# mickgordinier/DPX_GPU_Genomics_Project

Hardware: AMD Instinct MI355X
Metric: GCUPS (higher is better)
Workload: dtype int16; 1 GPU; LSW 10000-pair 1024x1024 batch per GPU, int16 score matrix written to HBM; algorithm=LSW, pairs_per_gpu=10000, query_len=1024, reference_len=1024, match=3, mismatch=-1, gap=-2, parallelism=1 GPU, world_size=1, tune_placement=True, cells_per_gpu=10485760000, matrix_bytes_per_gpu=22261760000, precondition_fills=78, kernel=k_linear_fill_pk, rows_per_lane=16

## Files before the change

### dpx_gpu_genomics_project_amd/csrc/dpx_capi.cpp

```cpp
#include <algorithm>
#include <cstdlib>
#include <cstring>
#include <mutex>
#include <string>
#include <vector>

#include "dpx_batch.h"

static std::mutex g_mu;
static int g_device = -1;

int dpx_host::bind_device(int device) {
    if (device < 0) {
        if (g_device < 0) {
            int rc = dpx_init(0);
            if (rc != DPX_OK) return rc;
        }
        device = g_device;
    }
    HIP_TRY(hipSetDevice(device));
    t_device = device;
    return DPX_OK;
}

// ... 525 lines not shown
    }
    if (r.dirs) return dpx_launch_fill_dir(b->dirArgs, b->kernelAlgo, b->R, s);
    if (r.split) return dpx_launch_fill_split(b->args, b->kernelAlgo, b->R, b->splitWaves, b->splitLds, s);
    hipStream_t side = s;
    bool forked = false;
    if (r.second != DPX_SECOND_NONE && r.main != DPX_MAIN_NONE && b->sideStream && b->evFork && b->evJoin) {
        hipError_t e = hipEventRecord(b->evFork, s);
        if (e == hipSuccess) e = hipStreamWaitEvent(b->sideStream, b->evFork, 0);
        if (e != hipSuccess) return e;
        side = b->sideStream;
        forked = true;
    }
    hipError_t e = launch_main(b, r, side);
    switch (e == hipSuccess ? r.second : DPX_SECOND_NONE) {
    case DPX_SECOND_NONE: break;
    case DPX_SECOND_PACKED: e = dpx_launch_fill_packed(b->pkArgs, b->kernelAlgo, b->R, b->pkLdsBytes, s); break;
    case DPX_SECOND_BANDED_PACKED: e = dpx_launch_banded_packed(b->pkArgs, b->R, b->pkLdsBytes, s); break;
    case DPX_SECOND_LANES:
        if (r.scoreTable) {
            dpx_subst_args ta = {b->pkArgs, table_ref(b)};
            ta.f.ldsPerWave = (uint32_t)dpx_plan_scoretab_lanes_lds(*b);
            e = dpx_launch_scoretab_lanes(ta, b->kernelAlgo, b->R, s);
            break;
        }
        e = dpx_launch_fill_lanes(b->pkArgs, b->kernelAlgo, b->R, b->store, b->pkLdsBytes, s);
        break;
    case DPX_SECOND_LANES_PK: e = dpx_launch_fill_lanes_packed(b->pkArgs, b->kernelAlgo, b->pkLdsBytes, s); break;
    }
    if (forked) {
        hipError_t j = hipEventRecord(b->evJoin, side);
        if (j == hipSuccess) j = hipStreamWaitEvent(s, b->evJoin, 0);
// ... 193 lines not shown
            len += snprintf(buf + len, cap - (size_t)len, "%s%.3f", k ? "," : "", r.candidatesMs[k]);
        if (r.candidatesMs.empty() && (size_t)len < cap) len += snprintf(buf + len, cap - (size_t)len, "untimed");
        if ((size_t)len < cap) len += snprintf(buf + len, cap - (size_t)len, " pool_fill_ms=");
        for (size_t k = 0; k < r.fillMs.size() && (size_t)len < cap; k++)
            len += snprintf(buf + len, cap - (size_t)len, "%s%.3f", k ? "," : "", r.fillMs[k]);
        if (r.fillMs.empty() && (size_t)len < cap) len += snprintf(buf + len, cap - (size_t)len, "unshopped");
        if (!r.kinds.empty() && (size_t)len < cap) {
            len += snprintf(buf + len, cap - (size_t)len, " pool_kinds=");
            for (size_t k = 0; k < r.kinds.size() && (size_t)len < cap; k++) len += snprintf(buf + len, cap - (size_t)len, "%s%s", k ? "," : "", r.kinds[k].c_str());
        }
        if (!r.ranges.empty() && (size_t)len < cap) {
            len += snprintf(buf + len, cap - (size_t)len, " pool_ranges=");
            for (size_t k = 0; k < r.ranges.size() && (size_t)len < cap; k++) len += snprintf(buf + len, cap - (size_t)len, "%s%s", k ? "," : "", r.ranges[k].c_str());
        }
    } else if (!b->dMat && len > 0 && (size_t)len < cap) len += snprintf(buf + len, cap - (size_t)len, " pool_addr=0x0");
    return DPX_OK;
}

int dpx_batch_info(dpx_batch *b, size_t *numPairs, uint64_t *cells, uint64_t *matrixBytes, uint64_t *algorithmicBytes) {
    if (!b) return DPX_ERR_INVALID;
    if (numPairs) *numPairs = b->numPairs;
    if (cells) *cells = b->cells;
    if (matrixBytes) *matrixBytes = b->matElems * sizeof(int16_t);
    if (algorithmicBytes) *algorithmicBytes = b->algBytes;
    return DPX_OK;
}


int dpx_align_batch(const dpx_params *params, const char *sequences, size_t numBytes, const dpx_seq_pair *pairs,
                    size_t numPairs, int32_t *scores, int32_t *endRow, int32_t *endCol, int16_t **H, int16_t **I,
// ... 44 lines not shown
```

### dpx_gpu_genomics_project_amd/csrc/dpx_host.cpp

```cpp
#include "dpx_host.h"

#include <cstdlib>
#include <cstring>
#include <mutex>

namespace dpx_host {

int hip_fail(hipError_t e, const char *what) {
    t_err = std::string(what) + ": " + hipGetErrorString(e);
    (void)hipGetLastError();
    return e == hipErrorOutOfMemory ? DPX_ERR_NOMEM : DPX_ERR_HIP;
}

static std::mutex g_knobsMu;
static Knobs g_knobs;
void refresh_knobs() {
    auto num = [](const char *name, int unset) { const char *e = getenv(name); return e ? atoi(e) : unset; };
    Knobs k;
    k.rowsPerLane = num("DPX_R", 0);
    k.packed = num("DPX_PACKED", -1);
    k.lanes = num("DPX_LANES", -1);
    k.lanesPk = num("DPX_LANES_PK", -1);
    k.split = num("DPX_SPLIT", -1);
    k.rowTags = num("DPX_ROW_TAGS", -1);
    k.rampLines = num("DPX_RAMP_LINES", -1);
    k.wavesPerBlock = num("DPX_WPB", 0);
    k.group = num("DPX_GROUP", 0);
    k.tbWalk = num("DPX_TB_WALK", -1);
    k.poolProbe = num("DPX_POOL_PROBE", -1);
    { const char *e = getenv("DPX_POOL"); k.poolMalloc = e && !strcmp(e, "malloc"); }
    { const long v = num("DPX_POOL_CHUNK_MB", 0); k.poolChunkBytes = v > 0 ? (size_t)v << 20 : 0; }
    { const char *e = getenv("DPX_POOL_GUARD"); k.poolGuard = !e ? 0 : !strcmp(e, "selftest") ? 2 : 1; }
    k.trace = getenv("DPX_TRACE") != nullptr;
    k.traceVmm = getenv("DPX_TRACE_VMM") != nullptr;
    std::lock_guard<std::mutex> lk(g_knobsMu);
    g_knobs = k;
}
Knobs knobs() { std::lock_guard<std::mutex> lk(g_knobsMu); return g_knobs; }

// ... 2 lines not shown
```

### dpx_gpu_genomics_project_amd/csrc/dpx_kernels.h

```cpp
#ifndef DPX_KERNELS_H
#define DPX_KERNELS_H

#include <hip/hip_runtime.h>
#include <stdint.h>

#include "dpx_layout.h"

#define DPX_K_LNW 0
#define DPX_K_LSW 1
#define DPX_K_ANW 2
#define DPX_K_BSW 3
#define DPX_K_ASW 4
#define DPX_K_BASW 5
#define DPX_K_ASG 6
#define DPX_K_BANW 7
#define DPX_K_BAXT 10


typedef struct dpx_fill_args {
    const char *seq;
    const dpx_pair_dev *pairs;
    const int32_t *order;
    const dpx_wave_desc *waves;
    int32_t numPairs;
// ... 6 lines not shown
    uint32_t ldsRefOff;
    uint32_t ldsQryOff;
    uint32_t ldsBufStride;
    int32_t rowTags;
    int32_t rampLines;
} dpx_fill_args;

hipError_t dpx_launch_fill(const dpx_fill_args &a, int algo, int R, bool store, size_t ldsBytes, hipStream_t stream);
hipError_t dpx_launch_fill_lanes(const dpx_fill_args &a, int algo, int R, bool store, size_t ldsBytes, hipStream_t stream);
hipError_t dpx_launch_affine_fill(const dpx_fill_args &a, int algo, int R, bool store, size_t ldsBytes, hipStream_t stream);
hipError_t dpx_launch_affine_lanes(const dpx_fill_args &a, int algo, int R, bool store, size_t ldsBytes, hipStream_t stream);
hipError_t dpx_launch_bsw_fill(const dpx_fill_args &a, int C, bool store, size_t ldsBytes, hipStream_t stream);
hipError_t dpx_launch_fill_lanes_packed(const dpx_fill_args &a, int algo, size_t ldsBytes, hipStream_t stream);
hipError_t dpx_launch_fill_split(const dpx_fill_args &a, int algo, int R, int waves, size_t ldsBytes, hipStream_t stream);
hipError_t dpx_launch_banded_packed(const dpx_fill_args &a, int C, size_t ldsBytes, hipStream_t stream);
hipError_t dpx_launch_fill_packed(const dpx_fill_args &a, int algo, int R, size_t ldsBytes, hipStream_t stream);
hipError_t dpx_launch_export(const int16_t *mat, const dpx_pair_dev &pr, int algo, int R, int planes, int plane, int gapOpen,
                             int gapExtend, int band, int16_t *out, hipStream_t stream);
hipError_t dpx_launch_traceback(const dpx_fill_args &a, int numPairs, int algo, int R, int planes, int walk,
                                const uint64_t *tbOff, char *tb, int32_t *tbLen, hipStream_t stream);
size_t dpx_out_scan_tiles(size_t numPairs);
hipError_t dpx_launch_output(const dpx_pair_dev *pairs, const int32_t *score, const int32_t *tbLen, const uint64_t *tbOff, const char *tb,
                             int numPairs, unsigned long long firstNumber, unsigned long long *tileSums, unsigned long long *outOff, char *out,
                             bool scanOnly, bool compactOnly, hipStream_t stream);
hipError_t dpx_launch_basw_fill(const dpx_fill_args &a, int C, bool store, size_t ldsBytes, hipStream_t stream);
hipError_t dpx_launch_basw_export(const int16_t *mat, const dpx_pair_dev &pr, int plane, int band, int16_t *out, hipStream_t stream);
hipError_t dpx_launch_basw_traceback(const dpx_fill_args &a, int numPairs, int walk, const uint64_t *tbOff, char *tb, int32_t *tbLen,
                                     hipStream_t stream);
hipError_t dpx_launch_banw_fill(const dpx_fill_args &a, int C, bool store, size_t ldsBytes, hipStream_t stream);
hipError_t dpx_launch_banw_export(const int16_t *mat, const dpx_pair_dev &pr, int plane, int band, int gapOpen, int gapExtend, int16_t *out,
                                  hipStream_t stream);
// ... 44 lines not shown
```

### dpx_gpu_genomics_project_amd/csrc/dpx_kernels.hip

```cpp
#include <hip/hip_runtime.h>
#include <stdint.h>

#include <type_traits>

#include "dpx_fill_common.hpp"
#include "dpx_kernels.h"
#include "dpx_layout.h"
#include "dpx_prims.hpp"

namespace {

using dpx::pack_lo16;
using dpx::wave_shr1;
using dpx::wave_shl1;
using dpx::s16x2;
using dpx::u16x2;
using dpx::as_s16x2;
using dpx::as_u16x2;
using dpx::as_u32;
using namespace dpx_dev;
using namespace dpx_fill;

template <int R, bool LOCAL>
struct LinState {
// ... 615 lines not shown
        __builtin_amdgcn_fence(__ATOMIC_RELEASE, "workgroup");
        int arrived = 0;
        if (lane == 0) arrived = __hip_atomic_fetch_add(&ctrl[16], 1, __ATOMIC_ACQ_REL, __HIP_MEMORY_SCOPE_WORKGROUP);
        arrived = __builtin_amdgcn_readfirstlane(arrived);
        if (arrived == W - 1 && lane == 0) {
            int bv = 0, br = 0, bc = 0;
            for (int k = 0; k < W; k++) {
                const int v = __hip_atomic_load(&result[4 * k], __ATOMIC_RELAXED, __HIP_MEMORY_SCOPE_WORKGROUP);
                if (v > bv) { bv = v; br = result[4 * k + 1]; bc = result[4 * k + 2]; }
            }
            a.score[p] = bv; a.endRow[p] = bv > 0 ? br : 0; a.endCol[p] = bv > 0 ? bc : 0;
        }
    }
}

template <int R>
struct PkState {
    uint32_t Hl[R];
    uint32_t qc[R];
    uint32_t rmax[R];
    uint32_t rcol[R];
    uint32_t dtop;
    uint32_t keyA, keyB;
};

template <int R, int TAG>
__device__ __forceinline__ uint32_t pk_row_tag(uint32_t h) {
    static_assert(TAG >= 0 && TAG < R && R <= 16, "inline constants");
    uint32_t r;
    asm("v_pk_mad_u16 %0, %1, %2, %3 op_sel_hi:[1,0,0]" : "=v"(r) : "v"(h), "n"(R), "n"(TAG));
    return r;
}
template <int R>
__device__ __forceinline__ uint32_t pk_row_tag_of(uint32_t h, const int r) {
#define DPX_TAG_CASE(k) case k: if constexpr (k < R) return pk_row_tag<R, (k < R ? R - 1 - k : 0)>(h); else return 0u;
    switch (r) {
        DPX_TAG_CASE(0) DPX_TAG_CASE(1) DPX_TAG_CASE(2) DPX_TAG_CASE(3) DPX_TAG_CASE(4) DPX_TAG_CASE(5) DPX_TAG_CASE(6) DPX_TAG_CASE(7)
        DPX_TAG_CASE(8) DPX_TAG_CASE(9) DPX_TAG_CASE(10) DPX_TAG_CASE(11) DPX_TAG_CASE(12) DPX_TAG_CASE(13) DPX_TAG_CASE(14) DPX_TAG_CASE(15)
    default: return 0u;
    }
#undef DPX_TAG_CASE
}

template <int R>
__device__ __forceinline__ void store_tile_pk(int16_t *dstA, int16_t *dstB, const uint32_t (&v)[R]) {
    if constexpr (R == 2) {
        *reinterpret_cast<uint32_t *>(dstA) = pk_hi16(v[0], v[1]);
        *reinterpret_cast<uint32_t *>(dstB) = pack_lo16((int)v[0], (int)v[1]);
    } else if constexpr (R == 4) {
        uint2 a, b;
        a.x = pk_hi16(v[0], v[1]); a.y = pk_hi16(v[2], v[3]);
        b.x = pack_lo16((int)v[0], (int)v[1]); b.y = pack_lo16((int)v[2], (int)v[3]);
        *reinterpret_cast<uint2 *>(dstA) = a;
        *reinterpret_cast<uint2 *>(dstB) = b;
    } else {
#pragma unroll
        for (int q = 0; q < R / 8; q++) {
            uint4 a, b;
            a.x = pk_hi16(v[8 * q + 0], v[8 * q + 1]); a.y = pk_hi16(v[8 * q + 2], v[8 * q + 3]);
            a.z = pk_hi16(v[8 * q + 4], v[8 * q + 5]); a.w = pk_hi16(v[8 * q + 6], v[8 * q + 7]);
            b.x = pack_lo16((int)v[8 * q + 0], (int)v[8 * q + 1]); b.y = pack_lo16((int)v[8 * q + 2], (int)v[8 * q + 3]);
            b.z = pack_lo16((int)v[8 * q + 4], (int)v[8 * q + 5]); b.w = pack_lo16((int)v[8 * q + 6], (int)v[8 * q + 7]);
            *reinterpret_cast<uint4 *>(dstA + q * 512) = a;
            *reinterpret_cast<uint4 *>(dstB + q * 512) = b;
        }
    }
}

template <int R, bool LOCAL, bool MASKED, bool WHOLE, bool TAGS = false, bool PARTIAL = false>
__device__ __forceinline__ void pk_step(PkState<R> &st, const int t, const int lane, const int n, const bool laneHasRows, const int nrows,
                                        const uint32_t matchP, const uint32_t negDeltaP, const uint32_t gapP, const uint32_t e0,
                                        const uint32_t rcP, uint32_t *edge, const bool writeEdge, int16_t *tileA, int16_t *tileB,
                                        const int storeLanes, const int rampLines) {
    const int j = t - lane + 1;
    const uint32_t upin = (uint32_t)wave_shr1((int)st.Hl[R - 1], (int)e0);
    bool active = true;
    if constexpr (MASKED) active = laneHasRows && (j >= 1) && (j <= n);
    if (active) {
        uint32_t u = upin, d = st.dtop;
        const uint32_t onesP = 0x00010001u;
        const uint32_t negj = 0xFFFFu - (uint32_t)j;
        uint32_t colMax = 0u;
#pragma unroll
        for (int r = 0; r < R; r++) {
            const uint32_t left = st.Hl[r];
            const uint32_t differs = dpx::pk_min_u16_raw(st.qc[r] ^ rcP, onesP);
            const s16x2 sc = as_s16x2(dpx::pk_mad_i16_raw(differs, negDeltaP, matchP));
            s16x2 h;
            if constexpr (LOCAL && TAGS) {
                h = dpx::pk_max(pk_gap_sat(u, left, gapP), (s16x2)(as_s16x2(d) + sc));
            } else {
                const s16x2 g = dpx::pk_max(as_s16x2(u), as_s16x2(left)) + as_s16x2(gapP);
                h = dpx::pk_max(g, (s16x2)(as_s16x2(d) + sc));
                if constexpr (LOCAL) h = dpx::pk_max(h, as_s16x2(0u));
            }
            d = left;
            u = as_u32(h);
            st.Hl[r] = u;
            if constexpr (LOCAL && TAGS) {
                uint32_t tg = pk_row_tag_of<R>(u, r);
                if constexpr (PARTIAL) tg = (r < nrows) ? tg : 0u;
                colMax = r == 0 ? tg : dpx::pk_max_u16_raw(colMax, tg);
            } else if constexpr (LOCAL) {
                st.rmax[r] = max(st.rmax[r], (u & 0xFFFF0000u) | negj);
                st.rcol[r] = max(st.rcol[r], (u << 16) | negj);
            }
        }
        if constexpr (LOCAL && TAGS) {
            st.keyA = max(st.keyA, (colMax & 0xFFFF0000u) | negj);
            st.keyB = max(st.keyB, (colMax << 16) | negj);
        }
        st.dtop = upin;
        if (writeEdge && lane == 63) edge[j] = st.Hl[R - 1];
        if constexpr (MASKED && !WHOLE) store_tile_pk<R>(tileA, tileB, st.Hl);
    }
    if constexpr (!MASKED || WHOLE) {
        bool doStore = lane < storeLanes;
        if constexpr (MASKED) doStore = doStore && ramp_stores<R>(lane, t, n, rampLines);
        if (doStore) store_tile_pk<R>(tileA, tileB, st.Hl);
    }
}

#ifndef DPX_PK_MIN_BLOCKS
#define DPX_PK_MIN_BLOCKS 1
#endif
template <int R, bool LOCAL, bool TAGS>
__global__ void __launch_bounds__(DPX_FILL_THREADS, DPX_PK_MIN_BLOCKS) k_linear_fill_pk(const dpx_fill_args a) {
    extern __shared__ __attribute__((aligned(16))) unsigned char smem[];
    const int lane = threadIdx.x & 63;
    const int wv = __builtin_amdgcn_readfirstlane(threadIdx.x >> 6);
    const int c = blockIdx.x * (int)a.wavesPerBlock + wv;
    if (c >= a.numPairs) return;
    const int pA = a.order[2 * c], pB = a.order[2 * c + 1];
    const dpx_pair_dev prA = a.pairs[pA], prB = a.pairs[pB];
    const int n = prA.n, m = prA.m;
    const unsigned char *refA = reinterpret_cast<const unsigned char *>(a.seq + prA.refIdx);
    const unsigned char *refB = reinterpret_cast<const unsigned char *>(a.seq + prB.refIdx);
    const unsigned char *qryA = reinterpret_cast<const unsigned char *>(a.seq + prA.qryIdx);
    const unsigned char *qryB = reinterpret_cast<const unsigned char *>(a.seq + prB.qryIdx);
    const int gap = a.gapOpen;
    const uint32_t matchP = ((uint32_t)(uint16_t)a.match << 16) | (uint16_t)a.match;
    const uint32_t negDeltaP = ((uint32_t)(uint16_t)(a.mismatch - a.match) << 16) | (uint16_t)(a.mismatch - a.match);
    const int gapK = (LOCAL && TAGS) ? -gap : gap;
    const uint32_t gapP = ((uint32_t)(uint16_t)gapK << 16) | (uint16_t)gapK;

    unsigned char *my = smem + (size_t)wv * a.ldsPerWave;
    uint32_t *edge = reinterpret_cast<uint32_t *>(my);
    uint16_t *refl = reinterpret_cast<uint16_t *>(my + a.ldsRefOff);
    for (int x = 4 * lane; x < n; x += 256) {
        const uint32_t a4 = load4(refA + x), b4 = load4(refB + x);
        uint2 w;
        w.x = __builtin_amdgcn_perm(a4, b4, 0x05010400u);
        w.y = __builtin_amdgcn_perm(a4, b4, 0x07030602u);
        *reinterpret_cast<uint2 *>(refl + 64 + x) = w;
    }
    for (int x = lane; x <= n + 1; x += 64) {
        const uint16_t b = (uint16_t)(LOCAL ? 0 : x * gap);
        edge[x] = ((uint32_t)b << 16) | b;
    }
    int16_t *HpA = a.mat + prA.matOff, *HpB = a.mat + prB.matOff;
    const int W = n + 63;
    const int S = dpx_tiled_stripes(m, R);
    int bestA = 0, browA = 0, bcolA = 0, bestB = 0, browB = 0, bcolB = 0;
    PkState<R> st;

    for (int k = 0; k < S; k++) {
        const int base = k * 64 * R;
        const int row0 = base + lane * R;
        const int nrows = min(max(m - row0, 0), R);
        const bool laneHasRows = nrows > 0;
// ... 309 lines not shown
    return dispatch_bool(algo == DPX_K_LSW, [&](auto local) {
        return launch_lds(k_linear_lanes_pk<decltype(local)::value>, grid, dim3(64 * wpb), ldsBytes, stream, a);
    });
}

hipError_t dpx_launch_fill_split(const dpx_fill_args &a, int algo, int R, int waves, size_t ldsBytes, hipStream_t stream) {
    if (a.numPairs <= 0) return hipSuccess;
    if (waves < 1 || waves > DPX_SPLIT_MAX_WAVES) return hipErrorInvalidValue;
    return dispatch_int<2, 4>(R, [&](auto r) {
        return dispatch_bool(algo == DPX_K_LSW, [&](auto local) {
            return launch_lds(k_linear_split<decltype(r)::value, decltype(local)::value>, dim3((unsigned)a.numPairs), dim3(64 * waves), ldsBytes, stream, a);
        });
    });
}

hipError_t dpx_launch_fill_packed(const dpx_fill_args &a, int algo, int R, size_t ldsBytes, hipStream_t stream) {
    if (a.numPairs <= 0) return hipSuccess;
    return dispatch_int<2, 4, 8, 16>(R, [&](auto r) {
        constexpr int kR = decltype(r)::value;
        if (algo != DPX_K_LSW) return launch_fill(k_linear_fill_pk<kR, false, false>, a, a, ldsBytes, stream);
        return a.rowTags ? launch_fill(k_linear_fill_pk<kR, true, true>, a, a, ldsBytes, stream)
                         : launch_fill(k_linear_fill_pk<kR, true, false>, a, a, ldsBytes, stream);
    });
}
```

### dpx_gpu_genomics_project_amd/csrc/dpx_plan.cpp

```cpp
#include "dpx_plan.h"

#include <algorithm>
#include <cstdio>
#include <cstdlib>
#include <cstring>
#include <numeric>
#include <utility>


constexpr size_t kLdsFloor = 36u * 1024u * (DPX_FILL_THREADS / 64) / 4;

bool is_affine(int algo) {
    return algo == DPX_ALGO_ANW || algo == DPX_ALGO_ASW || algo == DPX_ALGO_BASW || algo == DPX_ALGO_ASG || algo == DPX_ALGO_BANW ||
           algo == DPX_ALGO_BAXT;
}
bool is_banded(int algo) { return algo == DPX_ALGO_BSW || algo == DPX_ALGO_BASW || algo == DPX_ALGO_BANW || algo == DPX_ALGO_BAXT; }
bool is_banded_affine(int algo) { return algo == DPX_ALGO_BASW || algo == DPX_ALGO_BANW || algo == DPX_ALGO_BAXT; }
bool is_banw_layout(int algo) { return algo == DPX_ALGO_BANW || algo == DPX_ALGO_BAXT; }

int validate_params(const dpx_params *p) {
    if (!p) return DPX_ERR_INVALID;
    if ((p->algo < DPX_ALGO_LNW || p->algo > DPX_ALGO_BANW) && p->algo != DPX_ALGO_BAXT) return DPX_ERR_INVALID;
    if (is_banded(p->algo) && p->band < 1) return DPX_ERR_INVALID;
    const long long lim = 1ll << 20;
// ... 429 lines not shown
    a.ldsQryOff = banded ? 0u : (uint32_t)(l.edge * l.nEdges + l.ref);
    a.rampLines = kn.rampLines >= 0 ? kn.rampLines != 0 : p.numPairs >= 2048;
    if (p.split) {
        const SplitLds s = split_lds(p.maxN, p.splitWaves);
        a.ldsRefOff = 512u; a.ldsQryOff = (uint32_t)s.qryOff; a.ldsBufStride = (uint32_t)s.edgeStride;
    }
    dpx_fill_args &k = p.pkArgs;
    if (p.packed) {
        const PackedLds pl = packed_lds(banded, p.maxM, p.maxN);
        k = a;
        k.numPairs = (int32_t)p.nCouples; k.wavesPerBlock = fill_waves_per_block(p.nCouples, kn.wavesPerBlock);
        k.ldsPerWave = (uint32_t)pl.perWave; k.ldsRefOff = (uint32_t)pl.refOff;
        p.pkLdsBytes = pl.perWave * (DPX_FILL_THREADS / 64);
        k.rowTags = !banded && p.kernelAlgo == DPX_ALGO_LSW && top_score(p) * p.R + p.R - 1 <= 65535 && prm.gapOpen <= 0  &&
                    kn.rowTags != 0;
    } else if (p.lanePacked) {
        k = a;
        k.numPairs = (int32_t)p.nWaves; k.ldsPerWave = (uint32_t)(dpx_lanes_stage_bytes(p.kernelAlgo, p.R, p.store) + lanesRefArea);
        k.wavesPerBlock = is_affine(p.kernelAlgo) ? 1u : (kn.wavesPerBlock == 1 ? 1u : (uint32_t)dpx_lanes_waves_per_block(p.kernelAlgo));
        p.pkLdsBytes = (size_t)k.ldsPerWave * (size_t)k.wavesPerBlock;
        if (p.pkLdsBytes > kLdsMax) return DPX_ERR_UNSUPPORTED;
    }
    if (p.dirs) {
        const bool dirGlobal = l.dirPerWave > 64u * 1024u;
        if (dirGlobal) p.dirScratch = align_up(std::min<size_t>(std::max<size_t>(p.nSingles, 1), DPX_DIR_SCRATCH_SLOTS) * l.dirPerWave, 256);
        dpx_dir_args &d = p.dirArgs;
        d.numPairs = (int32_t)p.nSingles; d.match = prm.match; d.mismatch = prm.mismatch; d.gapOpen = prm.gapOpen; d.gapExtend = prm.gapExtend;
        d.ldsPerWave = (uint32_t)l.dirPerWave; d.ldsEdge2Off = (uint32_t)l.dirEdge; d.ldsRefOff = (uint32_t)(l.dirEdge * l.nEdges);
        d.wavesPerBlock = (dirGlobal || l.dirPerWave * 4 > kLdsMax) ? 1u : fill_waves_per_block(p.nSingles, kn.wavesPerBlock);
    }
// ... 60 lines not shown
        r.scoreTable = true;
        r.second = p.lanePacked ? DPX_SECOND_LANES : DPX_SECOND_NONE;
        if (!r.second || p.args.numPairs > 0) r.main = DPX_MAIN_FILL;
        r.kernel = p.lanePacked ? lanes[family] : fill[family];
    } else if (substAlphabet) {
        r.main = extension ? DPX_MAIN_ZSUB : DPX_MAIN_SUBST; r.kernel = extension ? DPX_K_ZSUB_FILL : DPX_K_SUBST_FILL;
    } else if (algo == DPX_ALGO_BAXT) {
        r.main = extension ? DPX_MAIN_ZEXT : DPX_MAIN_BAXT; r.kernel = extension ? DPX_K_ZEXT_FILL : DPX_K_BAXT_FILL;
    } else if (algo == DPX_ALGO_BANW) {
        r.main = DPX_MAIN_BANW; r.kernel = DPX_K_BANW_FILL;
    } else if (algo == DPX_ALGO_BASW) {
        r.main = DPX_MAIN_BASW; r.kernel = DPX_K_BASW_FILL;
    } else {
        const bool bsw = algo == DPX_ALGO_BSW;
        r.second = p.packed ? (bsw ? DPX_SECOND_BANDED_PACKED : DPX_SECOND_PACKED) : p.lanesPk ? DPX_SECOND_LANES_PK : p.lanePacked ? DPX_SECOND_LANES : DPX_SECOND_NONE;
        r.split = !r.second && p.split;
        if (r.second ? p.args.numPairs > 0 : !r.split) r.main = DPX_MAIN_FILL;
        r.kernel = bsw ? (p.packed ? DPX_K_BANDED_FILL_PK : DPX_K_BANDED_FILL)
                   : family ? (p.lanePacked ? lanes[family] : fill[family])
                   : p.packed ? DPX_K_LINEAR_FILL_PK : p.lanesPk ? DPX_K_LINEAR_LANES_PK : p.lanePacked ? DPX_K_LINEAR_LANES : p.split ? DPX_K_LINEAR_SPLIT : DPX_K_LINEAR_FILL;
    }
    r.extRecords = r.main == DPX_MAIN_ZEXT || r.main == DPX_MAIN_ZSUB || ((r.main == DPX_MAIN_BDX || r.main == DPX_MAIN_BD2) && extension);
    r.walk = p.bandLocal ? (p.twoPiece ? DPX_WALK_LB2 : DPX_WALK_BDL) : p.twoPiece ? DPX_WALK_BD2 : p.bandDirs ? DPX_WALK_BDIR : (substAlphabet && !p.dirs && !r.scoreTable) ? DPX_WALK_SUBST : algo == DPX_ALGO_BASW ? DPX_WALK_BASW : is_banw_layout(algo) ? DPX_WALK_BANW
             : p.dirs ? DPX_WALK_DIR : DPX_WALK_PLAIN;
    r.walkMode = (r.walk == DPX_WALK_BDL || r.walk == DPX_WALK_LB2 || r.walk == DPX_WALK_BD2 || r.walk == DPX_WALK_BDIR || r.walk == DPX_WALK_DIR) ? 0 : walk_mode(p, tbWalk);
    r.exportKind = is_banw_layout(algo)  ? DPX_EXPORT_BANW : algo == DPX_ALGO_BASW ? DPX_EXPORT_BASW : DPX_EXPORT_PLAIN;
    return r;
}

unsigned dpx_plan_bdx_waves(const dpx_plan &p, bool table) {
// ... 84 lines not shown
```

### dpx_gpu_genomics_project_amd/csrc/dpx_plan.h

```cpp
#ifndef DPX_PLAN_H
#define DPX_PLAN_H

#include <string>
#include <vector>

#include "../../include/dpx_align.h"
#include "dpx_dir.h"
#include "dpx_banddir.h"
#include "dpx_banddir2.h"

#pragma GCC visibility push(hidden)

struct Knobs {
    int rowsPerLane = 0;
    int packed = -1;
    int lanes = -1;
    int lanesPk = -1;
    int split = -1;
    int rowTags = -1;
    int rampLines = -1;
    int wavesPerBlock = 0;
    int group = 0;
    int tbWalk = -1;
    int poolProbe = -1;
    bool poolMalloc = false;
    size_t poolChunkBytes = 0;
    int poolGuard = 0;
    bool trace = false, traceVmm = false;
};

struct dpx_plan {
    dpx_params prm{}; unsigned flags = 0; size_t numPairs = 0;
    bool packed2 = false;
    int kernelAlgo = 0;
    int R = 8;
    int planes = 1;
    bool store = true;
    bool dirs = false;
    bool bandDirs = false;
    bool bandLocal = false;
    bool twoPiece = false;
    int32_t gapOpen2 = 0, gapExtend2 = 0;
    bool packed = false;
    bool split = false;
    bool lanePacked = false;
    bool lanesPk = false;
    int splitWaves = 0, maxM = 0, maxN = 0;
    size_t splitLds = 0;
    uint64_t cells = 0, matElems = 0, algBytes = 0, bandCells = 0;
    std::vector<dpx_pair_dev> pairs;
    std::vector<int32_t> singles;
    std::vector<int32_t> couples;
    std::vector<dpx_wave_desc> waves;
    std::vector<uint64_t> tbOff;
    size_t seqLo = 0, seqHi = 0;
    size_t packedDwords = 0, packedCopy = 0;
    size_t dirScratch = 0;
    dpx_fill_args args{};
    dpx_fill_args pkArgs{};
    dpx_dir_args dirArgs{};
    size_t ldsBytes = 0, pkLdsBytes = 0;
// ... 16 lines not shown
    DPX_K_ZEXT_FILL, DPX_K_SUBST_FILL, DPX_K_ZSUB_FILL, DPX_K_BDIR_FILL, DPX_K_BDX_FILL, DPX_K_BD2_FILL,
    DPX_K_LINEAR_DIR, DPX_K_AFFINE_DIR, DPX_K_ASW_DIR, DPX_K_ASG_DIR, DPX_K_BDL_FILL, DPX_K_BDLT_FILL, DPX_K_COUNT
};
enum dpx_main_launch { DPX_MAIN_NONE, DPX_MAIN_FILL, DPX_MAIN_BASW, DPX_MAIN_BANW, DPX_MAIN_BAXT, DPX_MAIN_ZEXT, DPX_MAIN_SUBST, DPX_MAIN_ZSUB, DPX_MAIN_BDIR, DPX_MAIN_BDX, DPX_MAIN_BD2, DPX_MAIN_BDL, DPX_MAIN_BDLT };
constexpr dpx_fill_kernel DPX_K_LB2_FILL = static_cast<dpx_fill_kernel>(DPX_K_COUNT + 1);
constexpr dpx_main_launch DPX_MAIN_LB2 = static_cast<dpx_main_launch>(DPX_MAIN_BDLT + 1);
enum dpx_second_launch { DPX_SECOND_NONE, DPX_SECOND_PACKED, DPX_SECOND_BANDED_PACKED, DPX_SECOND_LANES, DPX_SECOND_LANES_PK };
enum dpx_walk_family { DPX_WALK_PLAIN, DPX_WALK_DIR, DPX_WALK_BASW, DPX_WALK_BANW, DPX_WALK_SUBST, DPX_WALK_BDIR, DPX_WALK_BD2, DPX_WALK_BDL, DPX_WALK_LB2 };
enum dpx_export_kind { DPX_EXPORT_PLAIN, DPX_EXPORT_BASW, DPX_EXPORT_BANW };
struct dpx_route {
    dpx_fill_kernel kernel;
    bool dirs, split;
    bool dirTable;
    bool scoreTable;
    dpx_second_launch second;
    dpx_main_launch main;
    bool ext;
    bool extRecords;
    dpx_walk_family walk;
    int walkMode;
    dpx_export_kind exportKind;
};
dpx_route dpx_plan_route(const dpx_plan &p, int tbWalk, int zdrop, int endBonus, int substAlphabet);
unsigned dpx_plan_bdx_waves(const dpx_plan &p, bool table);
unsigned dpx_plan_dirtab_waves(const dpx_plan &p);
size_t dpx_plan_scoretab_lds(const dpx_plan &p), dpx_plan_scoretab_lanes_lds(const dpx_plan &p);
unsigned dpx_plan_scoretab_waves(const dpx_plan &p);
bool dpx_plan_scoretab_fits(const dpx_plan &p, std::string &err);
const char *dpx_route_kernel_name(dpx_fill_kernel k);
const char *dpx_route_walk_name(dpx_walk_family walk, int walkMode);
// ... 6 lines not shown
```

Before: 3214 GCUPS.

## Add block-keyed packed LSW fill tracking per-row max over column blocks

Adds a new packed local Smith-Waterman fill kernel that, instead of updating a tagged max key for every cell, keeps a per-row running max across a block of G columns. It folds that into the best-score key only once per block, then recovers the exact end column afterwards by rescanning the stored score matrix for that block. The goal is to cut the per-cell ALU work of best-position tracking in the inner loop. In exchange it adds extra registers per row (bmax) and a small post-pass of atomic loads from HBM to find the column. The new path is enabled by default for LSW with R of 8 or 16 and a single stripe, and can be disabled with DPX_BLOCK_KEYS=0.

Result: no change. 3265 GCUPS (median of 6 runs) (+1.6%).

```diff
diff --git a/dpx_gpu_genomics_project_amd/csrc/dpx_capi.cpp b/dpx_gpu_genomics_project_amd/csrc/dpx_capi.cpp
--- a/dpx_gpu_genomics_project_amd/csrc/dpx_capi.cpp
+++ b/dpx_gpu_genomics_project_amd/csrc/dpx_capi.cpp
@@ -563,7 +563,7 @@
     hipError_t e = launch_main(b, r, side);
     switch (e == hipSuccess ? r.second : DPX_SECOND_NONE) {
     case DPX_SECOND_NONE: break;
-    case DPX_SECOND_PACKED: e = dpx_launch_fill_packed(b->pkArgs, b->kernelAlgo, b->R, b->pkLdsBytes, s); break;
+    case DPX_SECOND_PACKED: e = dpx_launch_fill_packed(b->pkArgs, b->kernelAlgo, b->R, r.blockKeys, b->pkLdsBytes, s); break;
     case DPX_SECOND_BANDED_PACKED: e = dpx_launch_banded_packed(b->pkArgs, b->R, b->pkLdsBytes, s); break;
     case DPX_SECOND_LANES:
         if (r.scoreTable) {
@@ -787,6 +787,8 @@
             for (size_t k = 0; k < r.ranges.size() && (size_t)len < cap; k++) len += snprintf(buf + len, cap - (size_t)len, "%s%s", k ? "," : "", r.ranges[k].c_str());
         }
     } else if (!b->dMat && len > 0 && (size_t)len < cap) len += snprintf(buf + len, cap - (size_t)len, " pool_addr=0x0");
+    if (len > 0 && (size_t)len < cap)
+        len += snprintf(buf + len, cap - (size_t)len, " block_keys=%d", dpx_plan_route(*b, knobs().tbWalk, b->zdrop, b->endBonus, b->substAlphabet).blockKeys);
     return DPX_OK;
 }
 
diff --git a/dpx_gpu_genomics_project_amd/csrc/dpx_host.cpp b/dpx_gpu_genomics_project_amd/csrc/dpx_host.cpp
--- a/dpx_gpu_genomics_project_amd/csrc/dpx_host.cpp
+++ b/dpx_gpu_genomics_project_amd/csrc/dpx_host.cpp
@@ -23,6 +23,7 @@
     k.lanesPk = num("DPX_LANES_PK", -1);
     k.split = num("DPX_SPLIT", -1);
     k.rowTags = num("DPX_ROW_TAGS", -1);
+    k.blockKeys = num("DPX_BLOCK_KEYS", -1);
     k.rampLines = num("DPX_RAMP_LINES", -1);
     k.wavesPerBlock = num("DPX_WPB", 0);
     k.group = num("DPX_GROUP", 0);
diff --git a/dpx_gpu_genomics_project_amd/csrc/dpx_kernels.h b/dpx_gpu_genomics_project_amd/csrc/dpx_kernels.h
--- a/dpx_gpu_genomics_project_amd/csrc/dpx_kernels.h
+++ b/dpx_gpu_genomics_project_amd/csrc/dpx_kernels.h
@@ -44,7 +44,8 @@
 hipError_t dpx_launch_fill_lanes_packed(const dpx_fill_args &a, int algo, size_t ldsBytes, hipStream_t stream);
 hipError_t dpx_launch_fill_split(const dpx_fill_args &a, int algo, int R, int waves, size_t ldsBytes, hipStream_t stream);
 hipError_t dpx_launch_banded_packed(const dpx_fill_args &a, int C, size_t ldsBytes, hipStream_t stream);
-hipError_t dpx_launch_fill_packed(const dpx_fill_args &a, int algo, int R, size_t ldsBytes, hipStream_t stream);
+hipError_t dpx_launch_fill_packed(const dpx_fill_args &a, int algo, int R, int blockKeys, size_t ldsBytes, hipStream_t stream);
+hipError_t dpx_launch_fill_pkb(const dpx_fill_args &a, int R, int blockKeys, size_t ldsBytes, hipStream_t stream);
 hipError_t dpx_launch_export(const int16_t *mat, const dpx_pair_dev &pr, int algo, int R, int planes, int plane, int gapOpen,
                              int gapExtend, int band, int16_t *out, hipStream_t stream);
 hipError_t dpx_launch_traceback(const dpx_fill_args &a, int numPairs, int algo, int R, int planes, int walk,
diff --git a/dpx_gpu_genomics_project_amd/csrc/dpx_kernels.hip b/dpx_gpu_genomics_project_amd/csrc/dpx_kernels.hip
--- a/dpx_gpu_genomics_project_amd/csrc/dpx_kernels.hip
+++ b/dpx_gpu_genomics_project_amd/csrc/dpx_kernels.hip
@@ -653,112 +653,7 @@
     }
 }
 
-template <int R>
-struct PkState {
-    uint32_t Hl[R];
-    uint32_t qc[R];
-    uint32_t rmax[R];
-    uint32_t rcol[R];
-    uint32_t dtop;
-    uint32_t keyA, keyB;
-};
-
-template <int R, int TAG>
-__device__ __forceinline__ uint32_t pk_row_tag(uint32_t h) {
-    static_assert(TAG >= 0 && TAG < R && R <= 16, "inline constants");
-    uint32_t r;
-    asm("v_pk_mad_u16 %0, %1, %2, %3 op_sel_hi:[1,0,0]" : "=v"(r) : "v"(h), "n"(R), "n"(TAG));
-    return r;
-}
-template <int R>
-__device__ __forceinline__ uint32_t pk_row_tag_of(uint32_t h, const int r) {
-#define DPX_TAG_CASE(k) case k: if constexpr (k < R) return pk_row_tag<R, (k < R ? R - 1 - k : 0)>(h); else return 0u;
-    switch (r) {
-        DPX_TAG_CASE(0) DPX_TAG_CASE(1) DPX_TAG_CASE(2) DPX_TAG_CASE(3) DPX_TAG_CASE(4) DPX_TAG_CASE(5) DPX_TAG_CASE(6) DPX_TAG_CASE(7)
-        DPX_TAG_CASE(8) DPX_TAG_CASE(9) DPX_TAG_CASE(10) DPX_TAG_CASE(11) DPX_TAG_CASE(12) DPX_TAG_CASE(13) DPX_TAG_CASE(14) DPX_TAG_CASE(15)
-    default: return 0u;
-    }
-#undef DPX_TAG_CASE
-}
-
-template <int R>
-__device__ __forceinline__ void store_tile_pk(int16_t *dstA, int16_t *dstB, const uint32_t (&v)[R]) {
-    if constexpr (R == 2) {
-        *reinterpret_cast<uint32_t *>(dstA) = pk_hi16(v[0], v[1]);
-        *reinterpret_cast<uint32_t *>(dstB) = pack_lo16((int)v[0], (int)v[1]);
-    } else if constexpr (R == 4) {
-        uint2 a, b;
-        a.x = pk_hi16(v[0], v[1]); a.y = pk_hi16(v[2], v[3]);
-        b.x = pack_lo16((int)v[0], (int)v[1]); b.y = pack_lo16((int)v[2], (int)v[3]);
-        *reinterpret_cast<uint2 *>(dstA) = a;
-        *reinterpret_cast<uint2 *>(dstB) = b;
-    } else {
-#pragma unroll
-        for (int q = 0; q < R / 8; q++) {
-            uint4 a, b;
-            a.x = pk_hi16(v[8 * q + 0], v[8 * q + 1]); a.y = pk_hi16(v[8 * q + 2], v[8 * q + 3]);
-            a.z = pk_hi16(v[8 * q + 4], v[8 * q + 5]); a.w = pk_hi16(v[8 * q + 6], v[8 * q + 7]);
-            b.x = pack_lo16((int)v[8 * q + 0], (int)v[8 * q + 1]); b.y = pack_lo16((int)v[8 * q + 2], (int)v[8 * q + 3]);
-            b.z = pack_lo16((int)v[8 * q + 4], (int)v[8 * q + 5]); b.w = pack_lo16((int)v[8 * q + 6], (int)v[8 * q + 7]);
-            *reinterpret_cast<uint4 *>(dstA + q * 512) = a;
-            *reinterpret_cast<uint4 *>(dstB + q * 512) = b;
-        }
-    }
-}
-
-template <int R, bool LOCAL, bool MASKED, bool WHOLE, bool TAGS = false, bool PARTIAL = false>
-__device__ __forceinline__ void pk_step(PkState<R> &st, const int t, const int lane, const int n, const bool laneHasRows, const int nrows,
-                                        const uint32_t matchP, const uint32_t negDeltaP, const uint32_t gapP, const uint32_t e0,
-                                        const uint32_t rcP, uint32_t *edge, const bool writeEdge, int16_t *tileA, int16_t *tileB,
-                                        const int storeLanes, const int rampLines) {
-    const int j = t - lane + 1;
-    const uint32_t upin = (uint32_t)wave_shr1((int)st.Hl[R - 1], (int)e0);
-    bool active = true;
-    if constexpr (MASKED) active = laneHasRows && (j >= 1) && (j <= n);
-    if (active) {
-        uint32_t u = upin, d = st.dtop;
-        const uint32_t onesP = 0x00010001u;
-        const uint32_t negj = 0xFFFFu - (uint32_t)j;
-        uint32_t colMax = 0u;
-#pragma unroll
-        for (int r = 0; r < R; r++) {
-            const uint32_t left = st.Hl[r];
-            const uint32_t differs = dpx::pk_min_u16_raw(st.qc[r] ^ rcP, onesP);
-            const s16x2 sc = as_s16x2(dpx::pk_mad_i16_raw(differs, negDeltaP, matchP));
-            s16x2 h;
-            if constexpr (LOCAL && TAGS) {
-                h = dpx::pk_max(pk_gap_sat(u, left, gapP), (s16x2)(as_s16x2(d) + sc));
-            } else {
-                const s16x2 g = dpx::pk_max(as_s16x2(u), as_s16x2(left)) + as_s16x2(gapP);
-                h = dpx::pk_max(g, (s16x2)(as_s16x2(d) + sc));
-                if constexpr (LOCAL) h = dpx::pk_max(h, as_s16x2(0u));
-            }
-            d = left;
-            u = as_u32(h);
-            st.Hl[r] = u;
-            if constexpr (LOCAL && TAGS) {
-                uint32_t tg = pk_row_tag_of<R>(u, r);
-                if constexpr (PARTIAL) tg = (r < nrows) ? tg : 0u;
-                colMax = r == 0 ? tg : dpx::pk_max_u16_raw(colMax, tg);
-            } else if constexpr (LOCAL) {
-                st.rmax[r] = max(st.rmax[r], (u & 0xFFFF0000u) | negj);
-                st.rcol[r] = max(st.rcol[r], (u << 16) | negj);
-            }
-        }
-        if constexpr (LOCAL && TAGS) {
-            st.keyA = max(st.keyA, (colMax & 0xFFFF0000u) | negj);
-            st.keyB = max(st.keyB, (colMax << 16) | negj);
-        }
-        st.dtop = upin;
-        if (writeEdge && lane == 63) edge[j] = st.Hl[R - 1];
-        if constexpr (MASKED && !WHOLE) store_tile_pk<R>(tileA, tileB, st.Hl);
-    }
-    if constexpr (!MASKED || WHOLE) {
-        bool doStore = lane < storeLanes;
-        if constexpr (MASKED) doStore = doStore && ramp_stores<R>(lane, t, n, rampLines);
-        if (doStore) store_tile_pk<R>(tileA, tileB, st.Hl);
-    }
-}
+#include "dpx_pk_step.inc"
 
 #ifndef DPX_PK_MIN_BLOCKS
 #define DPX_PK_MIN_BLOCKS 1
@@ -786,13 +681,7 @@
     unsigned char *my = smem + (size_t)wv * a.ldsPerWave;
     uint32_t *edge = reinterpret_cast<uint32_t *>(my);
     uint16_t *refl = reinterpret_cast<uint16_t *>(my + a.ldsRefOff);
-    for (int x = 4 * lane; x < n; x += 256) {
-        const uint32_t a4 = load4(refA + x), b4 = load4(refB + x);
-        uint2 w;
-        w.x = __builtin_amdgcn_perm(a4, b4, 0x05010400u);
-        w.y = __builtin_amdgcn_perm(a4, b4, 0x07030602u);
-        *reinterpret_cast<uint2 *>(refl + 64 + x) = w;
-    }
+    DPX_PK_STAGE_REFS(refl, refA, refB, n, lane)
     for (int x = lane; x <= n + 1; x += 64) {
         const uint16_t b = (uint16_t)(LOCAL ? 0 : x * gap);
         edge[x] = ((uint32_t)b << 16) | b;
@@ -1132,8 +1021,12 @@
     });
 }
 
-hipError_t dpx_launch_fill_packed(const dpx_fill_args &a, int algo, int R, size_t ldsBytes, hipStream_t stream) {
+hipError_t dpx_launch_fill_packed(const dpx_fill_args &a, int algo, int R, int blockKeys, size_t ldsBytes, hipStream_t stream) {
     if (a.numPairs <= 0) return hipSuccess;
+    if (blockKeys) {
+        if (algo != DPX_K_LSW) return hipErrorInvalidValue;
+        return dpx_launch_fill_pkb(a, R, blockKeys, ldsBytes, stream);
+    }
     return dispatch_int<2, 4, 8, 16>(R, [&](auto r) {
         constexpr int kR = decltype(r)::value;
         if (algo != DPX_K_LSW) return launch_fill(k_linear_fill_pk<kR, false, false>, a, a, ldsBytes, stream);
diff --git a/dpx_gpu_genomics_project_amd/csrc/dpx_pk_step.inc b/dpx_gpu_genomics_project_amd/csrc/dpx_pk_step.inc
--- /dev/null
+++ b/dpx_gpu_genomics_project_amd/csrc/dpx_pk_step.inc
@@ -0,0 +1,118 @@
+template <int R>
+struct PkState {
+    uint32_t Hl[R];
+    uint32_t qc[R];
+    uint32_t rmax[R];
+    uint32_t rcol[R];
+    uint32_t dtop;
+    uint32_t keyA, keyB;
+    uint32_t bmax[R];
+};
+
+template <int R, int TAG>
+__device__ __forceinline__ uint32_t pk_row_tag(uint32_t h) {
+    static_assert(TAG >= 0 && TAG < R && R <= 16, "inline constants");
+    uint32_t r;
+    asm("v_pk_mad_u16 %0, %1, %2, %3 op_sel_hi:[1,0,0]" : "=v"(r) : "v"(h), "n"(R), "n"(TAG));
+    return r;
+}
+template <int R>
+__device__ __forceinline__ uint32_t pk_row_tag_of(uint32_t h, const int r) {
+#define DPX_TAG_CASE(k) case k: if constexpr (k < R) return pk_row_tag<R, (k < R ? R - 1 - k : 0)>(h); else return 0u;
+    switch (r) {
+        DPX_TAG_CASE(0) DPX_TAG_CASE(1) DPX_TAG_CASE(2) DPX_TAG_CASE(3) DPX_TAG_CASE(4) DPX_TAG_CASE(5) DPX_TAG_CASE(6) DPX_TAG_CASE(7)
+        DPX_TAG_CASE(8) DPX_TAG_CASE(9) DPX_TAG_CASE(10) DPX_TAG_CASE(11) DPX_TAG_CASE(12) DPX_TAG_CASE(13) DPX_TAG_CASE(14) DPX_TAG_CASE(15)
+    default: return 0u;
+    }
+#undef DPX_TAG_CASE
+}
+
+template <int R>
+__device__ __forceinline__ void store_tile_pk(int16_t *dstA, int16_t *dstB, const uint32_t (&v)[R]) {
+    if constexpr (R == 2) {
+        *reinterpret_cast<uint32_t *>(dstA) = pk_hi16(v[0], v[1]);
+        *reinterpret_cast<uint32_t *>(dstB) = pack_lo16((int)v[0], (int)v[1]);
+    } else if constexpr (R == 4) {
+        uint2 a, b;
+        a.x = pk_hi16(v[0], v[1]); a.y = pk_hi16(v[2], v[3]);
+        b.x = pack_lo16((int)v[0], (int)v[1]); b.y = pack_lo16((int)v[2], (int)v[3]);
+        *reinterpret_cast<uint2 *>(dstA) = a;
+        *reinterpret_cast<uint2 *>(dstB) = b;
+    } else {
+#pragma unroll
+        for (int q = 0; q < R / 8; q++) {
+            uint4 a, b;
+            a.x = pk_hi16(v[8 * q + 0], v[8 * q + 1]); a.y = pk_hi16(v[8 * q + 2], v[8 * q + 3]);
+            a.z = pk_hi16(v[8 * q + 4], v[8 * q + 5]); a.w = pk_hi16(v[8 * q + 6], v[8 * q + 7]);
+            b.x = pack_lo16((int)v[8 * q + 0], (int)v[8 * q + 1]); b.y = pack_lo16((int)v[8 * q + 2], (int)v[8 * q + 3]);
+            b.z = pack_lo16((int)v[8 * q + 4], (int)v[8 * q + 5]); b.w = pack_lo16((int)v[8 * q + 6], (int)v[8 * q + 7]);
+            *reinterpret_cast<uint4 *>(dstA + q * 512) = a;
+            *reinterpret_cast<uint4 *>(dstB + q * 512) = b;
+        }
+    }
+}
+
+template <int R, bool LOCAL, bool MASKED, bool WHOLE, bool TAGS = false, bool PARTIAL = false, int BLOCK = 0>
+__device__ __forceinline__ void pk_step(PkState<R> &st, const int t, const int lane, const int n, const bool laneHasRows, const int nrows,
+                                        const uint32_t matchP, const uint32_t negDeltaP, const uint32_t gapP, const uint32_t e0,
+                                        const uint32_t rcP, uint32_t *edge, const bool writeEdge, int16_t *tileA, int16_t *tileB,
+                                        const int storeLanes, const int rampLines) {
+    const int j = t - lane + 1;
+    const uint32_t upin = (uint32_t)wave_shr1((int)st.Hl[R - 1], (int)e0);
+    bool active = true;
+    if constexpr (MASKED) active = laneHasRows && (j >= 1) && (j <= n);
+    if (active) {
+        uint32_t u = upin, d = st.dtop;
+        const uint32_t onesP = 0x00010001u;
+        const uint32_t negj = 0xFFFFu - (uint32_t)j;
+        uint32_t colMax = 0u;
+#pragma unroll
+        for (int r = 0; r < R; r++) {
+            const uint32_t left = st.Hl[r];
+            const uint32_t differs = dpx::pk_min_u16_raw(st.qc[r] ^ rcP, onesP);
+            const s16x2 sc = as_s16x2(dpx::pk_mad_i16_raw(differs, negDeltaP, matchP));
+            s16x2 h;
+            if constexpr (LOCAL && TAGS) {
+                h = dpx::pk_max(pk_gap_sat(u, left, gapP), (s16x2)(as_s16x2(d) + sc));
+            } else {
+                const s16x2 g = dpx::pk_max(as_s16x2(u), as_s16x2(left)) + as_s16x2(gapP);
+                h = dpx::pk_max(g, (s16x2)(as_s16x2(d) + sc));
+                if constexpr (LOCAL) h = dpx::pk_max(h, as_s16x2(0u));
+            }
+            d = left;
+            u = as_u32(h);
+            st.Hl[r] = u;
+            if constexpr (LOCAL && TAGS && BLOCK != 0) {
+                st.bmax[r] = BLOCK == 2 ? u : dpx::pk_max_u16_raw(st.bmax[r], u);
+            } else if constexpr (LOCAL && TAGS) {
+                uint32_t tg = pk_row_tag_of<R>(u, r);
+                if constexpr (PARTIAL) tg = (r < nrows) ? tg : 0u;
+                colMax = r == 0 ? tg : dpx::pk_max_u16_raw(colMax, tg);
+            } else if constexpr (LOCAL) {
+                st.rmax[r] = max(st.rmax[r], (u & 0xFFFF0000u) | negj);
+                st.rcol[r] = max(st.rcol[r], (u << 16) | negj);
+            }
+        }
+        if constexpr (LOCAL && TAGS && BLOCK == 0) {
+            st.keyA = max(st.keyA, (colMax & 0xFFFF0000u) | negj);
+            st.keyB = max(st.keyB, (colMax << 16) | negj);
+        }
+        st.dtop = upin;
+        if (writeEdge && lane == 63) edge[j] = st.Hl[R - 1];
+        if constexpr (MASKED && !WHOLE) store_tile_pk<R>(tileA, tileB, st.Hl);
+    }
+    if constexpr (!MASKED || WHOLE) {
+        bool doStore = lane < storeLanes;
+        if constexpr (MASKED) doStore = doStore && ramp_stores<R>(lane, t, n, rampLines);
+        if (doStore) store_tile_pk<R>(tileA, tileB, st.Hl);
+    }
+}
+
+#define DPX_PK_STAGE_REFS(refl, refA, refB, n, lane)                                                                                       \
+    for (int x = 4 * (lane); x < (n); x += 256) {      \
+        const uint32_t a4 = load4((refA) + x), b4 = load4((refB) + x);                                                                     \
+        uint2 w;                                                                                                                           \
+        w.x = __builtin_amdgcn_perm(a4, b4, 0x05010400u);                            \
+        w.y = __builtin_amdgcn_perm(a4, b4, 0x07030602u);                                                                                  \
+        *reinterpret_cast<uint2 *>((refl) + 64 + x) = w;                  \
+    }
diff --git a/dpx_gpu_genomics_project_amd/csrc/dpx_pkb_kernels.hip b/dpx_gpu_genomics_project_amd/csrc/dpx_pkb_kernels.hip
--- /dev/null
+++ b/dpx_gpu_genomics_project_amd/csrc/dpx_pkb_kernels.hip
@@ -0,0 +1,162 @@
+#include <hip/hip_runtime.h>
+#include <stdint.h>
+
+#include "dpx_fill_common.hpp"
+#include "dpx_kernels.h"
+#include "dpx_layout.h"
+#include "dpx_prims.hpp"
+
+namespace {
+
+using dpx::pack_lo16;
+using dpx::wave_shr1;
+using dpx::s16x2;
+using dpx::as_s16x2;
+using dpx::as_u32;
+using namespace dpx_dev;
+using namespace dpx_fill;
+
+#include "dpx_pk_step.inc"
+
+#ifndef DPX_PK_MIN_BLOCKS
+#define DPX_PK_MIN_BLOCKS 1
+#endif
+
+template <int R, bool PARTIAL>
+__device__ __forceinline__ void pk_block_end(PkState<R> &st, const int b, const int nrows) {
+    uint32_t colMax = 0u;
+#pragma unroll
+    for (int r = 0; r < R; r++) {
+        uint32_t tg = pk_row_tag_of<R>(st.bmax[r], r);
+        if constexpr (PARTIAL) tg = (r < nrows) ? tg : 0u;
+        colMax = r == 0 ? tg : dpx::pk_max_u16_raw(colMax, tg);
+    }
+    const uint32_t negb = 0xFFFFu - (uint32_t)b;
+    st.keyA = max(st.keyA, (colMax & 0xFFFF0000u) | negb);
+    st.keyB = max(st.keyB, (colMax << 16) | negb);
+}
+template <int R>
+__device__ __forceinline__ void pk_block_zero(PkState<R> &st) {
+#pragma unroll
+    for (int r = 0; r < R; r++) st.bmax[r] = 0u;
+}
+template <int G>
+__device__ __forceinline__ int pk_block_first_column(const int16_t *row, const size_t cs, const int n, const int lane, const int b, const int want) {
+    int v[G];
+#pragma unroll
+    for (int k = 0; k < G; k++) {
+        const int t = G * b + k, j = t - lane + 1;
+        v[k] = (j >= 1 && j <= n) ? (int)__hip_atomic_load(row + (size_t)t * cs, __ATOMIC_RELAXED, __HIP_MEMORY_SCOPE_AGENT) : -1;
+    }
+    int col = 0;
+#pragma unroll
+    for (int k = G - 1; k >= 0; k--) col = (v[k] == want) ? G * b + k - lane + 1 : col;
+    return col;
+}
+
+template <int R, int G>
+__global__ void __launch_bounds__(DPX_FILL_THREADS, DPX_PK_MIN_BLOCKS) k_linear_fill_pkb(const dpx_fill_args a) {
+    static_assert((R == 8 || R == 16) && (G == 8 || G == 16), "63 is the last step of a block");
+    extern __shared__ __attribute__((aligned(16))) unsigned char smem[];
+    const int lane = threadIdx.x & 63;
+    const int wv = __builtin_amdgcn_readfirstlane(threadIdx.x >> 6);
+    const int c = blockIdx.x * (int)a.wavesPerBlock + wv;
+    if (c >= a.numPairs) return;
+    const int pA = a.order[2 * c], pB = a.order[2 * c + 1];
+    const dpx_pair_dev prA = a.pairs[pA], prB = a.pairs[pB];
+    const int n = prA.n, m = prA.m;
+    const unsigned char *qryA = reinterpret_cast<const unsigned char *>(a.seq + prA.qryIdx);
+    const unsigned char *qryB = reinterpret_cast<const unsigned char *>(a.seq + prB.qryIdx);
+    const uint32_t matchP = ((uint32_t)(uint16_t)a.match << 16) | (uint16_t)a.match;
+    const uint32_t negDeltaP = ((uint32_t)(uint16_t)(a.mismatch - a.match) << 16) | (uint16_t)(a.mismatch - a.match);
+    const uint32_t gapP = ((uint32_t)(uint16_t)(-a.gapOpen) << 16) | (uint16_t)(-a.gapOpen);
+
+    uint16_t *refl = reinterpret_cast<uint16_t *>(smem + (size_t)wv * a.ldsPerWave + a.ldsRefOff);
+    const unsigned char *refA = reinterpret_cast<const unsigned char *>(a.seq + prA.refIdx);
+    const unsigned char *refB = reinterpret_cast<const unsigned char *>(a.seq + prB.refIdx);
+    DPX_PK_STAGE_REFS(refl, refA, refB, n, lane)
+    const int W = n + 63;
+    const int row0 = lane * R;
+    const int nrows = min(max(m - row0, 0), R);
+    const bool laneHasRows = nrows > 0;
+    PkState<R> st;
+    {
+        int qa[R], qb[R];
+        load_query_rows<R>(qa, qryA, row0, nrows);
+        load_query_rows<R>(qb, qryB, row0, nrows);
+#pragma unroll
+        for (int r = 0; r < R; r++) {
+            st.qc[r] = ((uint32_t)qa[r] << 16) | (uint32_t)qb[r];
+            st.Hl[r] = 0u;
+            st.bmax[r] = 0u;
+        }
+        st.keyA = st.keyB = 0u;
+        st.dtop = 0u;
+    }
+    const size_t csA = prA.chunkStride, csB = prB.chunkStride;
+    int16_t *tileA = a.mat + prA.matOff + (size_t)lane * 8, *tileB = a.mat + prB.matOff + (size_t)lane * 8;
+    const uint16_t *rp = refl + 64 - lane;
+    uint32_t rcN = rp[0];
+    const int storeLanes = store_lanes<R>(m);
+#define DPX_PKB_STEP(MASKED_, HASROWS_, PARTIAL_, BLOCK_)                                                                     \
+    {                                                                                                                 \
+        const uint32_t rc16 = rcN;                                                                                    \
+        rcN = rp[t + 1];                                                                                              \
+        const uint32_t rcP = __builtin_amdgcn_perm(0u, rc16, 0x0c010c00u);       \
+        pk_step<R, true, MASKED_, true, true, PARTIAL_, BLOCK_>(st, t, lane, n, HASROWS_, nrows, matchP, negDeltaP, gapP, 0u, rcP, nullptr, false, \
+                                   tileA + (size_t)t * csA, tileB + (size_t)t * csB, storeLanes, a.rampLines);       \
+    }
+#define DPX_PKB_TAIL(PARTIAL_)                                                                                        \
+    if ((t & (G - 1)) == G - 1) { pk_block_end<R, PARTIAL_>(st, t / G, nrows); pk_block_zero<R>(st); }
+    if (m == 64 * R && n >= 64) {
+        int t = 0;
+        for (; t < 63; t++) { DPX_PKB_STEP(true, true, false, 1) DPX_PKB_TAIL(false) }
+        { DPX_PKB_STEP(false, true, false, 1) DPX_PKB_TAIL(false) t++; }
+        for (; t + G <= n;) {
+            DPX_PKB_STEP(false, true, false, 2) t++;
+#pragma unroll
+            for (int k = 1; k < G; k++) { DPX_PKB_STEP(false, true, false, 1) t++; }
+            pk_block_end<R, false>(st, (t - 1) / G, nrows);
+        }
+        pk_block_zero<R>(st);
+        for (; t < n; t++) { DPX_PKB_STEP(false, true, false, 1) DPX_PKB_TAIL(false) }
+        for (; t < W; t++) { DPX_PKB_STEP(true, true, false, 1) DPX_PKB_TAIL(false) }
+    } else {
+        for (int t = 0; t < W; t++) { DPX_PKB_STEP(true, laneHasRows, true, 1) DPX_PKB_TAIL(true) }
+    }
+#undef DPX_PKB_TAIL
+#undef DPX_PKB_STEP
+    if (W & (G - 1)) {
+        if (m == 64 * R) pk_block_end<R, false>(st, (W - 1) / G, nrows);
+        else pk_block_end<R, true>(st, (W - 1) / G, nrows);
+    }
+
+    constexpr int TB = R == 16 ? 4 : 3;
+    const int bestA = (int)(st.keyA >> (16 + TB)), bestB = (int)(st.keyB >> (16 + TB));
+    const int rA = R - 1 - (int)((st.keyA >> 16) & (R - 1)), rB = R - 1 - (int)((st.keyB >> 16) & (R - 1));
+    const unsigned long long mineA = ((unsigned long long)(unsigned)bestA << 32) | (unsigned)(0x7FFFFFFF - (row0 + 1 + rA));
+    const unsigned long long mineB = ((unsigned long long)(unsigned)bestB << 32) | (unsigned)(0x7FFFFFFF - (row0 + 1 + rB));
+    const unsigned long long topA = wave_max_u64(mineA), topB = wave_max_u64(mineB);
+    asm volatile("s_waitcnt vmcnt(0)" ::: "memory");
+    if ((int)(topA >> 32) == 0) { if (lane == 0) { a.score[pA] = 0; a.endRow[pA] = 0; a.endCol[pA] = 0; } }
+    else if (mineA == topA) {
+        a.score[pA] = bestA; a.endRow[pA] = row0 + 1 + rA;
+        a.endCol[pA] = pk_block_first_column<G>(tileA - (size_t)lane * 8 + dpx_tile_off(R, 0, lane, rA), csA, n, lane, 0xFFFF - (int)(st.keyA & 0xFFFFu), bestA);
+    }
+    if ((int)(topB >> 32) == 0) { if (lane == 0) { a.score[pB] = 0; a.endRow[pB] = 0; a.endCol[pB] = 0; } }
+    else if (mineB == topB) {
+        a.score[pB] = bestB; a.endRow[pB] = row0 + 1 + rB;
+        a.endCol[pB] = pk_block_first_column<G>(tileB - (size_t)lane * 8 + dpx_tile_off(R, 0, lane, rB), csB, n, lane, 0xFFFF - (int)(st.keyB & 0xFFFFu), bestB);
+    }
+}
+
+}
+
+hipError_t dpx_launch_fill_pkb(const dpx_fill_args &a, int R, int blockKeys, size_t ldsBytes, hipStream_t stream) {
+    if (!a.rowTags) return hipErrorInvalidValue;
+    return dispatch_int<8, 16>(R, [&](auto r) {
+        return dispatch_int<8, 16>(blockKeys, [&](auto g) {
+            return launch_fill(k_linear_fill_pkb<decltype(r)::value, decltype(g)::value>, a, a, ldsBytes, stream);
+        });
+    });
+}
diff --git a/dpx_gpu_genomics_project_amd/csrc/dpx_plan.cpp b/dpx_gpu_genomics_project_amd/csrc/dpx_plan.cpp
--- a/dpx_gpu_genomics_project_amd/csrc/dpx_plan.cpp
+++ b/dpx_gpu_genomics_project_amd/csrc/dpx_plan.cpp
@@ -467,6 +467,7 @@
         p.pkLdsBytes = pl.perWave * (DPX_FILL_THREADS / 64);
         k.rowTags = !banded && p.kernelAlgo == DPX_ALGO_LSW && top_score(p) * p.R + p.R - 1 <= 65535 && prm.gapOpen <= 0  &&
                     kn.rowTags != 0;
+        p.blockKeys = (k.rowTags && (p.R == 8 || p.R == 16) && dpx_tiled_stripes(p.maxM, p.R) == 1 && kn.blockKeys != 0) ? (kn.blockKeys == 16 ? 16 : 8) : 0;
     } else if (p.lanePacked) {
         k = a;
         k.numPairs = (int32_t)p.nWaves; k.ldsPerWave = (uint32_t)(dpx_lanes_stage_bytes(p.kernelAlgo, p.R, p.store) + lanesRefArea);
@@ -557,6 +558,7 @@
     } else {
         const bool bsw = algo == DPX_ALGO_BSW;
         r.second = p.packed ? (bsw ? DPX_SECOND_BANDED_PACKED : DPX_SECOND_PACKED) : p.lanesPk ? DPX_SECOND_LANES_PK : p.lanePacked ? DPX_SECOND_LANES : DPX_SECOND_NONE;
+        r.blockKeys = r.second == DPX_SECOND_PACKED ? p.blockKeys : 0;
         r.split = !r.second && p.split;
         if (r.second ? p.args.numPairs > 0 : !r.split) r.main = DPX_MAIN_FILL;
         r.kernel = bsw ? (p.packed ? DPX_K_BANDED_FILL_PK : DPX_K_BANDED_FILL)
diff --git a/dpx_gpu_genomics_project_amd/csrc/dpx_plan.h b/dpx_gpu_genomics_project_amd/csrc/dpx_plan.h
--- a/dpx_gpu_genomics_project_amd/csrc/dpx_plan.h
+++ b/dpx_gpu_genomics_project_amd/csrc/dpx_plan.h
@@ -18,6 +18,7 @@
     int lanesPk = -1;
     int split = -1;
     int rowTags = -1;
+    int blockKeys = -1;
     int rampLines = -1;
     int wavesPerBlock = 0;
     int group = 0;
@@ -45,6 +46,7 @@
     bool split = false;
     bool lanePacked = false;
     bool lanesPk = false;
+    int blockKeys = 0;
     int splitWaves = 0, maxM = 0, maxN = 0;
     size_t splitLds = 0;
     uint64_t cells = 0, matElems = 0, algBytes = 0, bandCells = 0;
@@ -91,6 +93,7 @@
     bool dirTable;
     bool scoreTable;
     dpx_second_launch second;
+    int blockKeys;
     dpx_main_launch main;
     bool ext;
     bool extRecords;
```
